# bghira/SimpleTuner

Measured on AMD Instinct MI355X. Metric: training images/sec (whole node), Flux.1-dev LoRA r32 1024^2 train step, higher is better.
Workload: dtype bf16

## Files before the change

### simpletuner_amd/csrc/gemm.hip

```cpp
#include <stdlib.h>
#include <type_traits>
#include "common.h"

#define BK 64
#define EPI_SPLITK 100

#ifdef ST355_TRACE
#define TR_T0 40
#define TR_MARKS 12
__device__ uint64_t st355_trace_buf[2][TR_MARKS];
#define TR_DECL uint64_t tr_[TR_MARKS] = {}
#define TR(t, k)                                                  \
  do {                                                            \
    if ((t) == TR_T0) tr_[k] = __builtin_amdgcn_s_memtime();       \
  } while (0)
#define TR_FLUSH(wv, lane)                                                              \
  do {                                                                                  \
    if (blockIdx.x == 64 && (lane) == 0 && ((wv) & 3) == 0)                              \
      for (int k_ = 0; k_ < TR_MARKS; k_++) st355_trace_buf[(wv) >> 2][k_] = tr_[k_];    \
  } while (0)
#else
#define TR_DECL
#define TR(t, k)
#define TR_FLUSH(wv, lane)
// ... 605 lines not shown
#define P3_THREADS 512
#define P3_XBYTES (P3_BM * BK * 2)
#define P3_WBYTES (P3_BN * BK * 2)
#define P3_STAGE (P3_XBYTES + P3_WBYTES)
#define P3_LDS (3 * P3_STAGE)

template <int EPI>
__global__ void __launch_bounds__(P3_THREADS, 2) k_gemm_p3(GemmGroup g) {
  extern __shared__ __attribute__((aligned(16))) char smem[];
  const int tid = threadIdx.x;
  const int lane = tid & 63;
  const int wv = __builtin_amdgcn_readfirstlane(tid >> 6);
  const int wm = wv >> 1, wn = wv & 1;

  int id = xcd_remap(blockIdx.x, gridDim.x);
  const int pi = id >= g.tiles0 ? 1 : 0;
  if (pi) id -= g.tiles0;
  const GemmP& p0 = g.p[pi];
  const int nbm = (p0.M + P3_BM - 1) / P3_BM, nbn = (p0.N + P3_BN - 1) / P3_BN;
  int pm, pn;
  tile_coords(id, nbm, nbn, pm, pn);
  const int m0 = pm * P3_BM, n0 = pn * P3_BN;
  const GemmP p = seg_view(p0, m0);
  const int nt1 = p.K / BK;
  const int nt = nt1 + p.K2 / BK;

  const bf16* A1 = p.A; const bf16* B1 = p.B; const bf16* A2 = p.A2; const bf16* B2 = p.B2;
  const int64_t la2 = p.lda2, lb2 = p.ldb2;
  const int M = p.M, N = p.N;
  const int st_row = lane >> 3, st_cp = lane & 7;
  int64_t xo[4], wo[2];
  int xrow[4], wrow[2], xc[4], wc[2];
#pragma unroll
  for (int j = 0; j < 4; j++) {
    const int row = (wv * 4 + j) * 8 + st_row;
    xc[j] = (st_cp ^ ((row >> 1) & 7)) * 8;
    xrow[j] = min(m0 + row, M - 1);
    xo[j] = (int64_t)xrow[j] * p.lda + xc[j];
  }
#pragma unroll
  for (int j = 0; j < 2; j++) {
    const int row = (wv * 2 + j) * 8 + st_row;
    wc[j] = (st_cp ^ ((row >> 1) & 7)) * 8;
    wrow[j] = min(n0 + row, N - 1);
    wo[j] = (int64_t)wrow[j] * p.ldb + wc[j];
  }
  auto stage = [&](int t, int buf) {
    char* xs = smem + buf * P3_STAGE;
    char* ws = xs + P3_XBYTES;
    if (t < nt1) {
      const int k0 = t * BK;
#pragma unroll
      for (int j = 0; j < 4; j++) glds16(A1 + xo[j] + k0, xs + (wv * 4 + j) * 1024);
#pragma unroll
      for (int j = 0; j < 2; j++) glds16(B1 + wo[j] + k0, ws + (wv * 2 + j) * 1024);
    } else {
      const int k0 = (t - nt1) * BK;
#pragma unroll
      for (int j = 0; j < 4; j++) glds16(A2 + (int64_t)xrow[j] * la2 + xc[j] + k0, xs + (wv * 4 + j) * 1024);
#pragma unroll
      for (int j = 0; j < 2; j++) glds16(B2 + (int64_t)wrow[j] * lb2 + wc[j] + k0, ws + (wv * 2 + j) * 1024);
    }
  };

  int w_off[2], w_sw[2], x_off[2], x_sw[2];
#pragma unroll
  for (int i = 0; i < 2; i++) {
    const int wr = wn * 64 + i * 32 + (lane & 31);
    w_off[i] = wr * 128; w_sw[i] = (wr >> 1) & 7;
    const int xr = wm * 64 + i * 32 + (lane & 31);
    x_off[i] = xr * 128; x_sw[i] = (xr >> 1) & 7;
  }
  const int khalf = lane >> 5;
  f32x16 acc[2][2];
#pragma unroll
  for (int i = 0; i < 2; i++)
#pragma unroll
    for (int j = 0; j < 2; j++)
#pragma unroll
      for (int r = 0; r < 16; r++) acc[i][j][r] = 0.f;

  stage(0, 0);
  if (nt > 1) {
    stage(1, 1);
    asm volatile("s_waitcnt vmcnt(6)" ::: "memory");
  } else {
    asm volatile("s_waitcnt vmcnt(0)" ::: "memory");
  }
  __builtin_amdgcn_s_barrier();
  int cur = 0;
  for (int t = 0; t < nt; t++) {
    if (t + 2 < nt) stage(t + 2, cur == 0 ? 2 : cur - 1);
    const char* xs = smem + cur * P3_STAGE;
    mma_tile(xs, xs + P3_XBYTES, x_off, x_sw, w_off, w_sw, khalf, acc);
    if (t + 1 < nt) {
      if (t + 2 < nt) asm volatile("s_waitcnt vmcnt(6)" ::: "memory");
      else asm volatile("s_waitcnt vmcnt(0)" ::: "memory");
      asm volatile("s_waitcnt lgkmcnt(0)" ::: "memory");
      __builtin_amdgcn_s_barrier();
    }
    cur = (cur == 2) ? 0 : cur + 1;
  }
  gemm_epilogue<EPI>(p, acc, m0 + wm * 64, n0 + wn * 64, lane);
}

#define PP_BARRIER()                                   \
  do {                                                 \
    asm volatile("" ::: "memory");                     \
    __builtin_amdgcn_s_barrier();                      \
    asm volatile("" ::: "memory");                     \
  } while (0)

#define PQ_BM 256
#define PQ_BN 256
#define PQ_BK 64
#define PQ_THREADS 512
#define PQ_REGION 16384
#define PQ_BUF (4 * PQ_REGION)
#define PQ_LDS (8 * 64 * 272)
#ifndef PQ_BUFLD
#define PQ_BUFLD 1
#endif
#ifndef PQ_VM
#define PQ_VM 8
#endif
#ifndef PQ_ABL
#define PQ_ABL 0
#endif
#ifndef PQ_PRIO
#ifndef PQ_F8_MX
#define PQ_F8_MX 1
#endif
typedef int i32x8 __attribute__((ext_vector_type(8)));
__device__ __forceinline__ i32x8 frag32(const long* p) {
  i32x8 v;
#pragma unroll
  for (int q = 0; q < 4; q++) { v[2 * q] = (int)(p[q] & 0xffffffffl); v[2 * q + 1] = (int)(p[q] >> 32); }
  return v;
}
#define PQ_PRIO 1
#endif
#ifndef PQ_GL
#define PQ_GL 1
#endif

__device__ __forceinline__ void wait_vm_rt(int n) {
  if (n >= 8) asm volatile("s_waitcnt vmcnt(8)" ::: "memory");
  else if (n == 6) asm volatile("s_waitcnt vmcnt(6)" ::: "memory");
  else if (n == 4) asm volatile("s_waitcnt vmcnt(4)" ::: "memory");
  else if (n == 2) asm volatile("s_waitcnt vmcnt(2)" ::: "memory");
  else asm volatile("s_waitcnt vmcnt(0)" ::: "memory");
}

template <int EPI, bool TN, bool F8 = false, bool CONV = false, int SK = 0>
__global__ void __launch_bounds__(PQ_THREADS, 2) k_gemm_pq(GemmGroup g) {
  static_assert(!SK || (!TN && !F8 && !CONV && EPI != EPI_SPLITK), "the stream-K tail is built for the plain NT bf16 problems");
  constexpr int ES = F8 ? 1 : 2;
  constexpr int KSN = F8 ? 8 : 4;
  static_assert(!(F8 && TN), "fp8 weight gradients are not built");
  extern __shared__ __attribute__((aligned(16))) char smem[];
  const int tid = threadIdx.x;
  const int lane = tid & 63;
  const int wv = __builtin_amdgcn_readfirstlane(tid >> 6);
  const int wm = wv >> 2, wn = wv & 3;

  int slice = (EPI == EPI_SPLITK) ? blockIdx.x / g.tiles0 : 0;
  int id = (EPI == EPI_SPLITK) ? xcd_remap(blockIdx.x % g.tiles0, g.tiles0) : xcd_remap(blockIdx.x, SK ? min((int)gridDim.x, g.sk_first) : (int)gridDim.x);
  int sk_n = 1, sk_tl = 0;
  if (SK && (int)blockIdx.x >= g.sk_first) {
    const int l = blockIdx.x - g.sk_first;
    sk_n = SK;
    const int lq = __builtin_amdgcn_readfirstlane((l >> 3) / sk_n);
    slice = (l >> 3) - lq * sk_n;
    sk_tl = 8 * lq + (l & 7);
    if (sk_tl >= g.tiles0 - g.sk_first) return;
    id = g.sk_first + sk_tl;
  }
  const int pi = id >= g.tiles0 ? 1 : 0;
  if (pi) id -= g.tiles0;
  const GemmP& p = g.p[pi];
  const int nbm = (p.M + PQ_BM - 1) / PQ_BM, nbn = (p.N + PQ_BN - 1) / PQ_BN;
  const int wtaps = (TN && p.conv_taps == 9) ? 9 : 1;
  int pm, pn;
  tile_coords(id, nbm, nbn * wtaps, pm, pn, TN ? ST355_TILE_GROUP : tile_group_for(p.K + p.K2));
  const int wtap = pn / nbn;
  pn -= wtap * nbn;
  const int m0 = pm * PQ_BM, n0 = pn * PQ_BN;
  const int64_t segi = (!TN && !F8 && !CONV && p.seg_rows) ? __builtin_amdgcn_readfirstlane(m0 / p.seg_rows) : 0;
  const int nt_all = p.K / (PQ_BK * 2 / ES);
  const int per = (EPI == EPI_SPLITK) ? (nt_all + p.ksplit - 1) / p.ksplit : SK ? __builtin_amdgcn_readfirstlane((nt_all + sk_n - 1) / sk_n) : nt_all;
  const int t_first = slice * per;
  const int nt1 = (EPI == EPI_SPLITK || SK) ? max(0, min(nt_all, t_first + per) - t_first) : nt_all;
  const int nt = nt1 + ((EPI == EPI_SPLITK || (SK && slice != sk_n - 1)) ? 0 : p.K2 / PQ_BK);

  const bf16* A1 = p.A + segi * p.seg_xa; const bf16* B1 = p.B; const bf16* A2 = p.A2 + segi * p.seg_xa2; const bf16* B2 = p.B2;
  const int64_t la2 = p.lda2, lb2 = p.ldb2;
  const int M = p.M, N = p.N;
  const char* xbase = TN ? (const char*)A1 + (int64_t)m0 * 2 : (const char*)A1 + (int64_t)m0 * p.lda * ES;
  const char* wbase = TN ? (const char*)B1 + (int64_t)n0 * 2 + (int64_t)((wtap / 3) * p.conv_wp + (wtap % 3)) * (wtaps > 1 ? p.ldb * 2 : 0)
                         : (const char*)B1 + (int64_t)n0 * p.ldb * ES;
  const uint32_t lda_b = (uint32_t)p.lda * ES, ldb_b = (uint32_t)p.ldb * ES;
  const int64_t xk_step = TN ? (int64_t)PQ_BK * lda_b : PQ_BK * 2;
  const int64_t wk_step = TN ? (int64_t)PQ_BK * ldb_b : PQ_BK * 2;
  constexpr bool conv = CONV;
  static_assert(!(CONV && (TN || F8)), "conv mode is the NT bf16 form");
  if (!conv) xbase += t_first * xk_step;
  wbase += t_first * wk_step;

  auto x_rel = [&](int lr, int r) { return min(m0 + (lr >> 6) * 128 + (lr & 63) + r * 64, M - 1) - m0; };
  auto w_rel = [&](int lr, int r) { return min(n0 + (lr >> 5) * 64 + (lr & 31) + r * 32, N - 1) - n0; };
  uint32_t xo[2][2], wo[2][2];
#pragma unroll
  for (int j = 0; j < 2; j++) {
    if (TN) {
      const int r4 = (wv * 2 + j) * 4 + (lane >> 4);
      const int cs = (lane & 15) ^ ((r4 & 3) << 2);
#pragma unroll
      for (int r = 0; r < 2; r++) {
        const int xc = min(m0 + (cs >> 3) * 128 + (cs & 7) * 8 + r * 64, M - 8) - m0;
        const int wc = min(n0 + (cs >> 2) * 64 + (cs & 3) * 8 + r * 32, N - 8) - n0;
        xo[r][j] = (uint32_t)r4 * lda_b + (uint32_t)(xc * 2);
        wo[r][j] = (uint32_t)r4 * ldb_b + (uint32_t)(wc * 2);
      }
    } else {
      const int lr = (wv * 2 + j) * 8 + (lane >> 3);
      const uint32_t scb = (uint32_t)(((lane & 7) ^ ((lr >> 1) & 7)) * 16);
#pragma unroll
      for (int r = 0; r < 2; r++) {
        xo[r][j] = (uint32_t)x_rel(lr, r) * lda_b + scb;
        wo[r][j] = (uint32_t)w_rel(lr, r) * ldb_b + scb;
      }
    }
  }
  auto stage_ext = [&](const bf16* base, int64_t ld, int row0, bool is_x, int r, int k0, char* dst) {
#pragma unroll
    for (int j = 0; j < 2; j++) {
      const int lr = (wv * 2 + j) * 8 + (lane >> 3);
      const int rel = is_x ? x_rel(lr, r) : w_rel(lr, r);
      glds16(base + (int64_t)(row0 + rel) * ld + ((lane & 7) ^ ((lr >> 1) & 7)) * 8 + k0, dst + j * 1024);
    }
  };
  const auto x_rsrc = __builtin_amdgcn_make_buffer_rsrc((void*)xbase, 0, 0x7FFFFFFF, 0x00020000);
  const auto w_rsrc = __builtin_amdgcn_make_buffer_rsrc((void*)wbase, 0, 0x7FFFFFFF, 0x00020000);
  auto stage_x = [&](int u, int r) {
    char* dst = smem + (u & 1) * PQ_BUF + r * PQ_REGION + wv * 2048;
    if (u < nt1) {
      const int x_ko = conv ? (int)(conv_koff(p, u + t_first, p.lda, PQ_BK) * 2)
                            : (int)(u * xk_step) + (TN ? (int)__umulhi((uint32_t)(u + t_first), p.tn_magic) * p.tn_skip_a : 0);
      if (PQ_BUFLD) {
#pragma unroll
        for (int j = 0; j < 2; j++)
          __builtin_amdgcn_raw_ptr_buffer_load_lds(x_rsrc, (__attribute__((address_space(3))) void*)(dst + j * 1024), 16, xo[r][j], x_ko, 0, 0);
        return;
      }
      const char* kb = xbase + x_ko;
#pragma unroll
      for (int j = 0; j < 2; j++) glds16((const bf16*)(kb + xo[r][j]), dst + j * 1024);
    } else {
      stage_ext(A2, la2, m0, true, r, (u - nt1) * PQ_BK, dst);
    }
  };
  auto stage_w = [&](int u, int r) {
    char* dst = smem + (u & 1) * PQ_BUF + (2 + r) * PQ_REGION + wv * 2048;
    if (u < nt1) {
      const int w_ko = (int)(u * wk_step) + (TN ? (int)__umulhi((uint32_t)(u + t_first), p.tn_magic) * p.tn_skip_b : 0);
      if (PQ_BUFLD) {
#pragma unroll
        for (int j = 0; j < 2; j++)
          __builtin_amdgcn_raw_ptr_buffer_load_lds(w_rsrc, (__attribute__((address_space(3))) void*)(dst + j * 1024), 16, wo[r][j], w_ko, 0, 0);
        return;
      }
      const char* kb = wbase + w_ko;
#pragma unroll
      for (int j = 0; j < 2; j++) glds16((const bf16*)(kb + wo[r][j]), dst + j * 1024);
    } else {
      stage_ext(B2, lb2, n0, false, r, (u - nt1) * PQ_BK, dst);
    }
  };
  auto refill = [&](int t, int ph, bool check) {
    if (PQ_ABL & 2) return;
    if (ph == 0) { if (!check || t + 1 < nt) stage_w(t + 1, 1); }
    else if (ph == 1) { if (!check || t + 1 < nt) stage_x(t + 1, 1); }
    else if (ph == 2) { if (!check || t + 2 < nt) stage_x(t + 2, 0); }
    else { if (!check || t + 2 < nt) stage_w(t + 2, 0); }
  };

  const int khalf = lane >> 5;
  const int l31 = lane & 31;
  int xk[4], wk[4];
#pragma unroll
  for (int ks = 0; ks < 4; ks++) {
    const int ch = ((2 * ks + khalf) ^ ((l31 >> 1) & 7)) << 4;
    xk[ks] = (wm * 64 + l31) * 128 + ch;
    wk[ks] = 2 * PQ_REGION + (wn * 32 + l31) * 128 + ch;
  }
  const int tg = lane >> 4, tti = (lane >> 2) & 3, tts = lane & 3;
  const int t_row = (8 * (tg >> 1) + tti) * 256 + (tts & 1) * 8;
  const int xt = t_row + (((wm * 8 + 2 * (tg & 1) + (tts >> 1)) ^ (tti << 2)) << 4);
  const int wt = 2 * PQ_REGION + t_row + (((wn * 4 + 2 * (tg & 1) + (tts >> 1)) ^ (tti << 2)) << 4);
  int xk8[8], wk8[8];
#pragma unroll
  for (int ks = 0; ks < 8; ks++) {
    const int chunk = PQ_F8_MX ? 4 * (ks >> 2) + 2 * khalf + ((ks & 3) >> 1) : ks;
    const int half8 = PQ_F8_MX ? (ks & 1) : khalf;
    const int ch = ((chunk ^ ((l31 >> 1) & 7)) << 4) + half8 * 8;
    xk8[ks] = (wm * 64 + l31) * 128 + ch;
    wk8[ks] = 2 * PQ_REGION + (wn * 32 + l31) * 128 + ch;
  }
  auto ld_x8 = [&](const char* base, int j, int ks) -> long { return *(const long*)(base + xk8[ks] + j * 4096); };
  auto ld_w8 = [&](const char* base, int ks) -> long { return *(const long*)(base + wk8[ks]); };
  auto ld_x = [&](const char* base, int j, int ks) -> bf16x8 {
    if (PQ_ABL & 1) { bf16x8 z; for (int q_ = 0; q_ < 8; q_++) z[q_] = (bf16)(float)(lane + j + ks); asm volatile("" : "+v"(z)); return z; }
    if (TN) { const char* q = base + (xt ^ (j << 6)) + ks * 4096; return lds_tr16x2(q, q + 1024); }
    return *(const bf16x8*)(base + xk[ks] + j * 4096);
  };
  auto ld_w = [&](const char* base, int ks) -> bf16x8 {
    if (PQ_ABL & 1) { bf16x8 z; for (int q_ = 0; q_ < 8; q_++) z[q_] = (bf16)(float)(lane + ks); asm volatile("" : "+v"(z)); return z; }
    if (TN) { const char* q = base + wt + ks * 4096; return lds_tr16x2(q, q + 1024); }
    return *(const bf16x8*)(base + wk[ks]);
  };
  f32x16 acc[2][4];
#pragma unroll
  for (int i = 0; i < 2; i++)
#pragma unroll
    for (int j = 0; j < 4; j++)
#pragma unroll
      for (int r = 0; r < 16; r++) acc[i][j][r] = 0.f;

  stage_x(0, 0); stage_w(0, 0); stage_w(0, 1); stage_x(0, 1);
  if (nt > 1) { stage_x(1, 0); stage_w(1, 0); }
  if (PQ_ABL & 2) wait_vm_rt(0); else
  wait_vm_rt(nt > 1 ? 8 : 4);
  PP_BARRIER();
  if (wm == 1) PP_BARRIER();

  bf16x8 xf[2][4], w0f[4], w1f[4];
  long xf8[2][8], w0f8[8], w1f8[8];
  const bool mma_live = !CONV || !p.skip_dead || (n0 + wn * 64 < N);
  TR_DECL;
#define PQ_MMA(WF, I, J0, T, PH)                                                                              \
  do {                                                                                                        \
    if (PQ_PRIO) __builtin_amdgcn_s_setprio(1);                                                               \
    if (F8 && PQ_F8_MX) {                                                                                     \
      _Pragma("unroll") for (int s2 = 0; s2 < 2; s2++)                                                        \
        _Pragma("unroll") for (int j = 0; j < 2; j++)                                                         \
          acc[I][J0 + j] = __builtin_amdgcn_mfma_scale_f32_32x32x64_f8f6f4(frag32(&WF##8[4 * s2]), frag32(&xf8[j][4 * s2]), acc[I][J0 + j], \
                                                                            0 , 1 , 0, 0x7f7f7f7f, 0, 0x7f7f7f7f); \
    } else if (F8) {                                                                                          \
      _Pragma("unroll") for (int ks = 0; ks < 8; ks++)                                                        \
        _Pragma("unroll") for (int j = 0; j < 2; j++)                                                         \
          acc[I][J0 + j] = __builtin_amdgcn_mfma_f32_32x32x16_fp8_bf8(WF##8[ks], xf8[j][ks], acc[I][J0 + j], 0, 0, 0); \
    } else if (!CONV || mma_live)                                                                             \
    _Pragma("unroll") for (int ks = 0; ks < 4; ks++) {                                                        \
      _Pragma("unroll") for (int j = 0; j < 2; j++)                                                           \
        acc[I][J0 + j] = __builtin_amdgcn_mfma_f32_32x32x16_bf16(WF[ks], xf[j][ks], acc[I][J0 + j], 0, 0, 0); \
      if (PQ_GL == 3 && ks == 1) { __builtin_amdgcn_sched_barrier(0); refill(T, PH, TAIL); __builtin_amdgcn_sched_barrier(0); } \
    }                                                                                                         \
    if (PQ_PRIO) __builtin_amdgcn_s_setprio(0);                                                               \
  } while (0)

  auto body = [&](int t, auto tail_c) {
    constexpr bool TAIL = decltype(tail_c)::value;
    const char* bf = smem + (t & 1) * PQ_BUF;
    const int rem = nt - 1 - t;
    TR(t, 0);
    if (PQ_GL == 0) refill(t, 0, TAIL);
#pragma unroll
    for (int j = 0; j < 2; j++)
#pragma unroll
      for (int ks = 0; ks < KSN; ks++) { if (F8) xf8[j][ks] = ld_x8(bf, j, ks); else xf[j][ks & 3] = ld_x(bf, j, ks & 3); }
#pragma unroll
    for (int ks = 0; ks < KSN; ks++) { if (F8) w0f8[ks] = ld_w8(bf, ks); else w0f[ks & 3] = ld_w(bf, ks & 3); }
    if (PQ_GL == 1) refill(t, 0, TAIL);
    TR(t, 1);
    if (!TAIL) wait_vm_rt(PQ_VM); else wait_vm_rt(rem >= 2 ? 8 : (rem == 1 ? 8 : 2));
    PP_BARRIER();
    TR(t, 2);
    PQ_MMA(w0f, 0, 0, t, 1);
    if (PQ_GL == 2) refill(t, 1, TAIL);
    TR(t, 3);
    PP_BARRIER();
    if (PQ_GL == 0) refill(t, 1, TAIL);
#pragma unroll
    for (int ks = 0; ks < KSN; ks++) { if (F8) w1f8[ks] = ld_w8(bf + PQ_REGION, ks); else w1f[ks & 3] = ld_w(bf + PQ_REGION, ks & 3); }
    if (PQ_GL == 1) refill(t, 1, TAIL);
    TR(t, 4);
    if (!TAIL) wait_vm_rt(PQ_VM); else wait_vm_rt(rem >= 2 ? 8 : (rem == 1 ? 8 : 0));
    PP_BARRIER();
    TR(t, 5);
    PQ_MMA(w1f, 1, 0, t, 2);
    if (PQ_GL == 2) refill(t, 2, TAIL);
    TR(t, 6);
    PP_BARRIER();
    if (PQ_GL == 0) refill(t, 2, TAIL);
#pragma unroll
    for (int j = 0; j < 2; j++)
#pragma unroll
      for (int ks = 0; ks < KSN; ks++) { if (F8) xf8[j][ks] = ld_x8(bf + PQ_REGION, j, ks); else xf[j][ks & 3] = ld_x(bf + PQ_REGION, j, ks & 3); }
    if (PQ_GL == 1) refill(t, 2, TAIL);
    TR(t, 7);
    if (!TAIL) wait_vm_rt(PQ_VM); else wait_vm_rt(rem >= 2 ? 8 : (rem == 1 ? 6 : 0));
    PP_BARRIER();
    TR(t, 8);
    PQ_MMA(w1f, 1, 2, t, 3);
    if (PQ_GL == 2) refill(t, 3, TAIL);
    TR(t, 9);
    PP_BARRIER();
    if (PQ_GL == 0) refill(t, 3, TAIL);
    if (PQ_GL == 1) refill(t, 3, TAIL);
    if (!TAIL) wait_vm_rt(PQ_VM); else wait_vm_rt(rem >= 2 ? 8 : (rem == 1 ? 4 : 0));
    PP_BARRIER();
    TR(t, 10);
    PQ_MMA(w0f, 0, 2, t + 1, 0);
    if (PQ_GL == 2) refill(t + 1, 0, TAIL);
    TR(t, 11);
    PP_BARRIER();
  };
  if (PQ_GL == 2 || PQ_GL == 3) refill(0, 0, true);
  int t = 0;
  for (; t < nt - 2; t++) body(t, std::false_type{});
  for (; t < nt; t++) body(t, std::true_type{});
#undef PQ_MMA
  TR_FLUSH(wv, lane);
  if (wm == 0) PP_BARRIER();
  if (SK && sk_n > 1) {
    float* slab = g.sk_ws + ((int64_t)sk_tl * (sk_n - 1)) * (PQ_BM * PQ_BN) + tid * 4;
    int* flag = g.sk_flags + sk_tl;
    if (slice < sk_n - 1) {
      slab += (int64_t)slice * (PQ_BM * PQ_BN);
#pragma unroll
      for (int i = 0; i < 2; i++)
#pragma unroll
        for (int j = 0; j < 4; j++)
#pragma unroll
          for (int a = 0; a < 4; a++) {
            f32x4 v;
#pragma unroll
            for (int b = 0; b < 4; b++) v[b] = acc[i][j][4 * a + b];
            *(f32x4*)(slab + ((i * 4 + j) * 4 + a) * (PQ_THREADS * 4)) = v;
          }
      asm volatile("s_waitcnt vmcnt(0)" ::: "memory");
      __syncthreads();
      if (tid == 0) __hip_atomic_fetch_add(flag, 1, __ATOMIC_RELAXED, __HIP_MEMORY_SCOPE_AGENT);
      return;
    }
    if (tid == 0)
      while (__hip_atomic_load(flag, __ATOMIC_RELAXED, __HIP_MEMORY_SCOPE_AGENT) < sk_n - 1) __builtin_amdgcn_s_sleep(4);
    __syncthreads();
    asm volatile("" ::: "memory");
#pragma unroll
    for (int i = 0; i < 2; i++)
#pragma unroll
      for (int j = 0; j < 4; j++) {
        f32x4 v[SK > 1 ? SK - 1 : 1][4];
#pragma unroll
        for (int k = 0; k < SK - 1; k++)
#pragma unroll
          for (int a = 0; a < 4; a++) v[k][a] = *(const f32x4*)(slab + (int64_t)k * (PQ_BM * PQ_BN) + ((i * 4 + j) * 4 + a) * (PQ_THREADS * 4));
#pragma unroll
        for (int k = 0; k < SK - 1; k++)
#pragma unroll
          for (int a = 0; a < 4; a++)
#pragma unroll
            for (int b = 0; b < 4; b++) acc[i][j][4 * a + b] += v[k][a][b];
        asm volatile("" ::: "memory");
      }
    if (tid == 0) __hip_atomic_store(flag, 0, __ATOMIC_RELAXED, __HIP_MEMORY_SCOPE_AGENT);
  }
  if (EPI == EPI_SPLITK) {
    GemmP ps = p;
    ps.partial = p.partial + (int64_t)slice * p.M * p.part_ld + (int64_t)wtap * p.N;
    ps.bias = nullptr;
    ps.conv_taps = 0;
    gemm_epilogue_lds<EPI, false, false>(ps, acc, m0 + wm * 128, n0 + wn * 64, lane, smem + wv * EPL_WAVE);
  } else if (wtaps > 1) {
    GemmP ps = p;
    ps.C = p.C + (int64_t)wtap * p.N;
    if (ps.aux_in) ps.aux_in = p.aux_in + (int64_t)wtap * p.N;
    ps.conv_taps = 0;
    gemm_epilogue_lds<EPI, false, false>(ps, acc, m0 + wm * 128, n0 + wn * 64, lane, smem + wv * EPL_WAVE);
  } else if (EPI == ST355_EPI_HEADS) {
    gemm_epilogue_heads(p, p.C + segi * p.seg_xc, acc, m0 + wm * 128, n0 + wn * 64, lane, smem + wv * EPL_WAVE);
  } else if (EPI == ST355_EPI_GEGLU) {
    gemm_epilogue_geglu(p, acc, m0 + wm * 128, n0 + wn * 64, lane, smem + wv * EPL_WAVE);
  } else if (EPI == ST355_EPI_GEGLU_GRAD) {
    gemm_epilogue_geglu_grad(p, acc, m0 + wm * 128, n0 + wn * 64, lane, smem + wv * EPL_WAVE);
  } else if (EPI == ST355_EPI_QK_NORM_ROPE) {
    if (n0 >= 2 * p.rH * 128) {
      gemm_epilogue_vdual(p, p.C + segi * p.seg_xc, acc, m0, n0, wm, wn, wv, lane, smem);
    } else {
      gemm_epilogue_qkrope(p, acc, m0, n0, wm, wn, wv, lane, smem);
    }
  } else if (!TN && !F8 && !CONV) {
    GemmP ps = p;
    ps.C = p.C + segi * p.seg_xc;
    ps.aux_in = p.aux_in + segi * p.seg_xin;
    ps.aux_out = p.aux_out + segi * p.seg_xout;
    if (epl_aligned(ps)) gemm_epilogue_lds<EPI, false, false>(ps, acc, m0 + wm * 128, n0 + wn * 64, lane, smem + wv * EPL_WAVE);
    else gemm_epilogue<EPI, 2, 4>(ps, acc, m0 + wm * 128, n0 + wn * 64, lane);
  } else if (epl_aligned(p)) gemm_epilogue_lds<EPI, CONV, F8>(p, acc, m0 + wm * 128, n0 + wn * 64, lane, smem + wv * EPL_WAVE);
  else gemm_epilogue<EPI, 2, 4>(p, acc, m0 + wm * 128, n0 + wn * 64, lane);
}

#define PZ_LDS (2 * PQ_BUF + 32768)
#define PZ_STAGE 8192

template <int EPI>
__device__ __forceinline__ void gemm_epilogue_lds8(const GemmP& p, f32x16 (&acc)[2][4], int mw0, int nw0, int lane, char* stage) {
  const int khalf = lane >> 5, l31 = lane & 31;
  const int rrow = lane >> 3, rc = lane & 7;
  const int n = nw0 + rc * 8;
  float bias8[8];
#pragma unroll
  for (int b = 0; b < 8; b++) bias8[b] = 0.f;
  if (p.bias) {
    const bf16x8 bv = *(const bf16x8*)(p.bias + n);
#pragma unroll
    for (int b = 0; b < 8; b++) bias8[b] = bf2f(bv[b]);
  }
  const int m_first = mw0 + rrow;
  constexpr bool GG = EPI == ST355_EPI_GEGLU_GRAD;
  const int nc = GG ? 2 * nw0 + 64 * (rc >> 2) + (rc & 3) * 8 : n;
  bf16* c_row = p.C + (int64_t)m_first * p.ldc + nc;
  const bf16* in_row = p.aux_in ? p.aux_in + (int64_t)m_first * p.ld_aux_in + nc : nullptr;
  bf16* out_row = p.aux_out ? p.aux_out + (int64_t)m_first * p.ld_aux_out + n : nullptr;
  const int64_t c_step = 8 * p.ldc, in_step = 8 * p.ld_aux_in, out_step = 8 * p.ld_aux_out;
  typedef __attribute__((address_space(3))) char lds_char;
  typedef __attribute__((address_space(3))) f32x4 lds_f32x4;
  const uint32_t stage_u = (uint32_t)(uintptr_t)(lds_char*)stage;
  const uint32_t wbase0 = stage_u + (uint32_t)(l31 * 256 + ((khalf ^ (l31 & 15)) << 4));
  const uint32_t rb = stage_u + (uint32_t)(rrow * 256);
  const uint32_t r_lo_e = rb + (uint32_t)((((2 * rc) ^ rrow)) << 4), r_hi_e = rb + (uint32_t)((((2 * rc + 1) ^ rrow)) << 4);
  const uint32_t r_lo_o = rb + (uint32_t)((((2 * rc) ^ (rrow | 8))) << 4), r_hi_o = rb + (uint32_t)((((2 * rc + 1) ^ (rrow | 8))) << 4);
  constexpr bool AUXIN = (EPI == ST355_EPI_GATE_RESIDUAL || EPI == ST355_EPI_ADD || EPI == ST355_EPI_MUL_GELU_GRAD || GG);
  bf16x8 auxv[2][4], gatev[2][4];
  const bf16* in_pre = in_row;
  int m_pre = m_first;
  auto preload = [&](bf16x8 (&av)[4], bf16x8 (&gv)[4]) {
#pragma unroll
    for (int it = 0; it < 4; it++) {
      if (AUXIN) av[it] = *(const bf16x8*)in_pre;
      if (EPI == ST355_EPI_GATE_RESIDUAL) gv[it] = *(const bf16x8*)(p.gate + (int64_t)(m_pre / p.rows_per_batch) * p.gate_stride + n);
      if (GG) gv[it] = *(const bf16x8*)(in_pre + 32);
      in_pre += in_step; m_pre += 8;
    }
  };
  if (AUXIN) preload(auxv[0], gatev[0]);
#pragma unroll
  for (int j = 0; j < 4; j++) {
    uint32_t wb = wbase0;
    asm volatile("" : "+v"(wb));
#pragma unroll
    for (int i = 0; i < 2; i++)
#pragma unroll
      for (int a = 0; a < 4; a++) {
        f32x4 v;
#pragma unroll
        for (int b = 0; b < 4; b++) v[b] = acc[i][j][4 * a + b];
        *(lds_f32x4*)(wb ^ (uint32_t)((i * 8 + 2 * a) << 4)) = v;
      }
    if (AUXIN && j < 3) preload(auxv[(j + 1) & 1], gatev[(j + 1) & 1]);
#pragma unroll
    for (int it = 0; it < 4; it++) {
      const f32x4 lo = *(const lds_f32x4*)(((it & 1) ? r_lo_o : r_lo_e) + (uint32_t)(it * 2048));
      const f32x4 hi = *(const lds_f32x4*)(((it & 1) ? r_hi_o : r_hi_e) + (uint32_t)(it * 2048));
      bf16* const c_ptr = c_row;
      bf16* const out_ptr = out_row;
      c_row += c_step; out_row += out_step;
      float v[8];
#pragma unroll
      for (int b = 0; b < 4; b++) { v[b] = lo[b] + bias8[b]; v[4 + b] = hi[b] + bias8[4 + b]; }
      if (EPI == ST355_EPI_GELU) {
        if (p.aux_out) {
          bf16x8 pre;
#pragma unroll
          for (int b = 0; b < 8; b++) pre[b] = f2bf(v[b]);
          *(bf16x8*)out_ptr = pre;
#pragma unroll
          for (int b = 0; b < 8; b++) v[b] = bf2f(pre[b]);
        }
#pragma unroll
        for (int b = 0; b < 8; b++) v[b] = gelu_tanh(v[b]);
      } else if (EPI == ST355_EPI_GATE_RESIDUAL) {
        if (p.aux_out) {
          bf16x8 yv;
#pragma unroll
          for (int b = 0; b < 8; b++) yv[b] = f2bf(v[b]);
          *(bf16x8*)out_ptr = yv;
        }
        const bf16x8 gv = gatev[j & 1][it];
        const bf16x8 rv = auxv[j & 1][it];
#pragma unroll
        for (int b = 0; b < 8; b++) v[b] = bf2f(rv[b]) + bf2f(gv[b]) * v[b];
      } else if (EPI == ST355_EPI_ADD) {
        const bf16x8 rv = auxv[j & 1][it];
#pragma unroll
        for (int b = 0; b < 8; b++) v[b] += bf2f(rv[b]);
      } else if (EPI == ST355_EPI_MUL_GELU_GRAD) {
        const bf16x8 hv = auxv[j & 1][it];
#pragma unroll
        for (int b = 0; b < 8; b++) v[b] *= gelu_tanh_grad(bf2f(hv[b]));
      }
      if (GG) {
        const bf16x8 vv = auxv[j & 1][it], gv = gatev[j & 1][it];
        bf16x8 dv, dg;
#pragma unroll
        for (int b = 0; b < 8; b++) {
          const float d = bf2f(f2bf(v[b]));
          const float g = bf2f(gv[b]);
          dv[b] = f2bf(d * gelu_erf(g));
          dg[b] = f2bf(d * bf2f(vv[b]) * gelu_erf_grad(g));
        }
        *(bf16x8*)c_ptr = dv;
        *(bf16x8*)(c_ptr + 32) = dg;
        continue;
      }
      bf16x8 o;
#pragma unroll
      for (int b = 0; b < 8; b++) o[b] = f2bf(v[b]);
      *(bf16x8*)c_ptr = o;
    }
  }
}

template <int EPI>
__global__ void __launch_bounds__(PQ_THREADS, 2) k_gemm_pz(GemmP p, int ntiles) {
  extern __shared__ __attribute__((aligned(16))) char smem[];
  const int tid = threadIdx.x;
  const int lane = tid & 63;
  const int wv = __builtin_amdgcn_readfirstlane(tid >> 6);
  const int wm = wv >> 2, wn = wv & 3;
  const int nbm = p.M / PQ_BM, nbn = p.N / PQ_BN;
  const int nt1 = p.K / PQ_BK;
  const int nt = nt1 + p.K2 / PQ_BK;
  const int G = gridDim.x;
  const uint32_t lda_b = (uint32_t)p.lda * 2, ldb_b = (uint32_t)p.ldb * 2;
  const int64_t la2 = p.lda2, lb2 = p.ldb2;

  struct Tile { int m0, n0; const char* xb; const char* wb; const bf16* a2; const bf16* b2; int64_t segi; };
  auto tile_at = [&](int id) {
    Tile t;
    int pm, pn;
    tile_coords(id, nbm, nbn, pm, pn);
    t.m0 = __builtin_amdgcn_readfirstlane(pm * PQ_BM);
    t.n0 = __builtin_amdgcn_readfirstlane(pn * PQ_BN);
    t.segi = p.seg_rows ? (int64_t)__builtin_amdgcn_readfirstlane(t.m0 / p.seg_rows) : 0;
    t.xb = (const char*)(p.A + t.segi * p.seg_xa) + (int64_t)t.m0 * lda_b;
    t.wb = (const char*)p.B + (int64_t)t.n0 * ldb_b;
    t.a2 = p.A2 + t.segi * p.seg_xa2 + (int64_t)t.m0 * la2;
    t.b2 = p.B2 + (int64_t)t.n0 * lb2;
    return t;
  };

  int tile_id = xcd_remap(blockIdx.x, G);
  Tile cur = tile_at(tile_id);
  int par = 0;
  bool first = true;

  while (true) {
    int ln = lane;
    asm volatile("" : "+v"(ln));
    uint32_t xo[2][2], wo[2][2];
#pragma unroll
    for (int j = 0; j < 2; j++) {
      const int lr = (wv * 2 + j) * 8 + (ln >> 3);
      const uint32_t scb = (uint32_t)(((ln & 7) ^ ((lr >> 1) & 7)) * 16);
#pragma unroll
      for (int r = 0; r < 2; r++) {
        xo[r][j] = (uint32_t)((lr >> 6) * 128 + (lr & 63) + r * 64) * lda_b + scb;
        wo[r][j] = (uint32_t)((lr >> 5) * 64 + (lr & 31) + r * 32) * ldb_b + scb;
      }
    }
    const int khalf = ln >> 5;
    const int l31 = ln & 31;
    int xk[4], wk[4];
#pragma unroll
    for (int ks = 0; ks < 4; ks++) {
      const int ch = ((2 * ks + khalf) ^ ((l31 >> 1) & 7)) << 4;
      xk[ks] = (wm * 64 + l31) * 128 + ch;
      wk[ks] = 2 * PQ_REGION + (wn * 32 + l31) * 128 + ch;
    }
    auto ld_x = [&](const char* base, int j, int ks) -> bf16x8 { return *(const bf16x8*)(base + xk[ks] + j * 4096); };
    auto ld_w = [&](const char* base, int ks) -> bf16x8 { return *(const bf16x8*)(base + wk[ks]); };
    const bool has_next = tile_id + G < ntiles;
    const Tile nxt = has_next ? tile_at(tile_id + G) : cur;
    const auto x_rsrc = __builtin_amdgcn_make_buffer_rsrc((void*)cur.xb, 0, 0x7FFFFFFF, 0x00020000);
    const auto w_rsrc = __builtin_amdgcn_make_buffer_rsrc((void*)cur.wb, 0, 0x7FFFFFFF, 0x00020000);
    const auto xn_rsrc = __builtin_amdgcn_make_buffer_rsrc((void*)nxt.xb, 0, 0x7FFFFFFF, 0x00020000);
    const auto wn_rsrc = __builtin_amdgcn_make_buffer_rsrc((void*)nxt.wb, 0, 0x7FFFFFFF, 0x00020000);

    auto stage_x = [&](int u, int r, int mode) {
      char* dst = smem + (((u & 1) ^ par) * PQ_BUF) + r * PQ_REGION + wv * 2048;
      const bool nx = mode == 1 && u >= nt;
      const int uu = nx ? u - nt : u;
      if (uu < nt1) {
#pragma unroll
        for (int j = 0; j < 2; j++)
          __builtin_amdgcn_raw_ptr_buffer_load_lds(nx ? xn_rsrc : x_rsrc, (__attribute__((address_space(3))) void*)(dst + j * 1024), 16, xo[r][j], uu * (PQ_BK * 2), 0, 0);
      } else {
        const bf16* base = nx ? nxt.a2 : cur.a2;
#pragma unroll
        for (int j = 0; j < 2; j++) {
          const int lr = (wv * 2 + j) * 8 + (ln >> 3);
          glds16(base + (int64_t)((lr >> 6) * 128 + (lr & 63) + r * 64) * la2 + ((ln & 7) ^ ((lr >> 1) & 7)) * 8 + (uu - nt1) * PQ_BK, dst + j * 1024);
        }
      }
    };
    auto stage_w = [&](int u, int r, int mode) {
      char* dst = smem + (((u & 1) ^ par) * PQ_BUF) + (2 + r) * PQ_REGION + wv * 2048;
      const bool nx = mode == 1 && u >= nt;
      const int uu = nx ? u - nt : u;
      if (uu < nt1) {
#pragma unroll
        for (int j = 0; j < 2; j++)
          __builtin_amdgcn_raw_ptr_buffer_load_lds(nx ? wn_rsrc : w_rsrc, (__attribute__((address_space(3))) void*)(dst + j * 1024), 16, wo[r][j], uu * (PQ_BK * 2), 0, 0);
      } else {
        const bf16* base = nx ? nxt.b2 : cur.b2;
#pragma unroll
        for (int j = 0; j < 2; j++) {
          const int lr = (wv * 2 + j) * 8 + (ln >> 3);
          glds16(base + (int64_t)((lr >> 5) * 64 + (lr & 31) + r * 32) * lb2 + ((ln & 7) ^ ((lr >> 1) & 7)) * 8 + (uu - nt1) * PQ_BK, dst + j * 1024);
        }
      }
    };
    auto refill = [&](int t, int ph, int mode) {
      const int u = (ph < 2) ? t + 1 : t + 2;
      if (mode == 2 && u >= nt) return;
      if (ph == 0) stage_w(u, 1, mode);
      else if (ph == 1) stage_x(u, 1, mode);
      else if (ph == 2) stage_x(u, 0, mode);
      else stage_w(u, 0, mode);
    };

    f32x16 acc[2][4];
#pragma unroll
    for (int i = 0; i < 2; i++)
#pragma unroll
      for (int j = 0; j < 4; j++)
#pragma unroll
        for (int r = 0; r < 16; r++) acc[i][j][r] = 0.f;

    if (first) {
      stage_x(0, 0, 0); stage_w(0, 0, 0); stage_w(0, 1, 0); stage_x(0, 1, 0);
      stage_x(1, 0, 0); stage_w(1, 0, 0);
      wait_vm_rt(8);
      PP_BARRIER();
    }
    if (wm == 1) PP_BARRIER();

    bf16x8 xf[2][4], w0f[4], w1f[4];
#define PZ_MMA(WF, I, J0)                                                                                     \
  do {                                                                                                        \
    __builtin_amdgcn_s_setprio(1);                                                                            \
    _Pragma("unroll") for (int ks = 0; ks < 4; ks++)                                                          \
      _Pragma("unroll") for (int j = 0; j < 2; j++)                                                           \
        acc[I][J0 + j] = __builtin_amdgcn_mfma_f32_32x32x16_bf16(WF[ks], xf[j][ks], acc[I][J0 + j], 0, 0, 0); \
    __builtin_amdgcn_s_setprio(0);                                                                            \
  } while (0)

    auto body = [&](int t, auto mode_c, auto firstk_c) {
      constexpr int MODE = decltype(mode_c)::value;
      constexpr bool FIRSTK = decltype(firstk_c)::value;
      const char* bf = smem + (((t & 1) ^ par) * PQ_BUF);
      const int rem = nt - 1 - t;
#pragma unroll
      for (int j = 0; j < 2; j++)
#pragma unroll
        for (int ks = 0; ks < 4; ks++) xf[j][ks] = ld_x(bf, j, ks);
#pragma unroll
      for (int ks = 0; ks < 4; ks++) w0f[ks] = ld_w(bf, ks);
      refill(t, 0, MODE);
      if (MODE != 2) { if (!FIRSTK) wait_vm_rt(8); } else wait_vm_rt(rem >= 1 ? 8 : 2);
      PP_BARRIER();
      PZ_MMA(w0f, 0, 0);
      PP_BARRIER();
#pragma unroll
      for (int ks = 0; ks < 4; ks++) w1f[ks] = ld_w(bf + PQ_REGION, ks);
      refill(t, 1, MODE);
      if (MODE != 2) { if (!FIRSTK) wait_vm_rt(8); } else wait_vm_rt(rem >= 1 ? 8 : 0);
      PP_BARRIER();
      PZ_MMA(w1f, 1, 0);
      PP_BARRIER();
#pragma unroll
      for (int j = 0; j < 2; j++)
#pragma unroll
        for (int ks = 0; ks < 4; ks++) xf[j][ks] = ld_x(bf + PQ_REGION, j, ks);
      refill(t, 2, MODE);
      if (MODE != 2) wait_vm_rt(8); else wait_vm_rt(rem >= 1 ? 6 : 0);
      PP_BARRIER();
      PZ_MMA(w1f, 1, 2);
      PP_BARRIER();
      refill(t, 3, MODE);
      if (MODE != 2) wait_vm_rt(8); else wait_vm_rt(rem >= 1 ? 4 : 0);
      PP_BARRIER();
      PZ_MMA(w0f, 0, 2);
      PP_BARRIER();
    };
    int t = 0;
    if (!first) { body(0, std::integral_constant<int, 0>{}, std::true_type{}); t = 1; }
    for (; t < nt - 2; t++) body(t, std::integral_constant<int, 0>{}, std::false_type{});
    for (; t < nt; t++) body(t, std::integral_constant<int, 1>{}, std::false_type{});
#undef PZ_MMA
    if (wm == 0) PP_BARRIER();
    wait_vm_rt(4);
    {
      GemmP ps = p;
      ps.C = p.C + cur.segi * p.seg_xc;
      ps.aux_in = p.aux_in ? p.aux_in + cur.segi * p.seg_xin : nullptr;
      ps.aux_out = p.aux_out ? p.aux_out + cur.segi * p.seg_xout : nullptr;
      char* const lastbuf = smem + ((((nt - 1) & 1) ^ par) * PQ_BUF);
      char* const stg = wv < 2 ? lastbuf + PQ_REGION + wv * PZ_STAGE : (wv < 4 ? lastbuf + 3 * PQ_REGION + (wv - 2) * PZ_STAGE : smem + 2 * PQ_BUF + (wv - 4) * PZ_STAGE);
      int le = lane;
      asm volatile("" : "+v"(le));
      gemm_epilogue_lds8<EPI>(ps, acc, cur.m0 + wm * 128, cur.n0 + wn * 64, le, stg);
    }
    if (!has_next) { wait_vm_rt(0); break; }
    PP_BARRIER();
    par ^= (nt & 1);
    tile_id += G;
    cur = nxt;
    first = false;
  }
}

#define S2_BM 128
#define S2_BN 128
#define S2_THREADS 256
#define S2_TILE (128 * BK * 2)
#define S2_STAGE (2 * S2_TILE)
#define S2_LDS (2 * S2_STAGE)

template <int EPI>
__global__ void __launch_bounds__(S2_THREADS, 2) k_gemm_s2(GemmP p_in) {
  extern __shared__ __attribute__((aligned(16))) char smem[];
  const int tid = threadIdx.x;
  const int lane = tid & 63;
  const int wv = __builtin_amdgcn_readfirstlane(tid >> 6);
  const int wm = wv >> 1, wn = wv & 1;
  const int nbm = (p_in.M + S2_BM - 1) / S2_BM, nbn = (p_in.N + S2_BN - 1) / S2_BN;
  int pm, pn;
  const int tiles = nbm * nbn;
  const int slice = (EPI == EPI_SPLITK) ? blockIdx.x / tiles : 0;
  tile_coords(xcd_remap((EPI == EPI_SPLITK) ? blockIdx.x % tiles : blockIdx.x, tiles), nbm, nbn, pm, pn);
  const int m0 = pm * S2_BM, n0 = pn * S2_BN;
  const GemmP p = seg_view(p_in, m0);
  const int nt1 = p.K / BK;
  const int per = (EPI == EPI_SPLITK) ? (nt1 + p.ksplit - 1) / p.ksplit : 0;
  const int t_first = (EPI == EPI_SPLITK) ? slice * per : 0;
  const int nt = (EPI == EPI_SPLITK) ? min(nt1, t_first + per) : nt1 + p.K2 / BK;
  const int st_row = lane >> 3, st_cp = lane & 7;
  auto stage = [&](int t, int buf) {
    const bf16* Ap; const bf16* Bp; int64_t la, lb; int k0;
    if (t < nt1) { Ap = p.A; la = p.lda; Bp = p.B; lb = p.ldb; k0 = t * BK; }
    else { Ap = p.A2; la = p.lda2; Bp = p.B2; lb = p.ldb2; k0 = (t - nt1) * BK; }
    const int64_t ka = (p.conv_taps && t < nt1) ? conv_koff(p, t, la, BK) : (int64_t)k0;
    char* xs = smem + buf * S2_STAGE;
    char* ws = xs + S2_TILE;
#pragma unroll
    for (int j = 0; j < 4; j++) {
      const int r0 = (wv * 4 + j) * 8;
      const int row = r0 + st_row;
      const int c = st_cp ^ ((row >> 1) & 7);
      glds16(Ap + (int64_t)min(m0 + row, p.M - 1) * la + ka + c * 8, xs + r0 * 128);
      glds16(Bp + (int64_t)min(n0 + row, p.N - 1) * lb + k0 + c * 8, ws + r0 * 128);
    }
  };
  int w_off[2], w_sw[2], x_off[2], x_sw[2];
#pragma unroll
  for (int i = 0; i < 2; i++) {
    const int wr = wn * 64 + i * 32 + (lane & 31);
    w_off[i] = wr * 128; w_sw[i] = (wr >> 1) & 7;
    const int xr = wm * 64 + i * 32 + (lane & 31);
    x_off[i] = xr * 128; x_sw[i] = (xr >> 1) & 7;
  }
  const int khalf = lane >> 5;
  f32x16 acc[2][2];
#pragma unroll
  for (int i = 0; i < 2; i++)
#pragma unroll
    for (int j = 0; j < 2; j++)
#pragma unroll
      for (int r = 0; r < 16; r++) acc[i][j][r] = 0.f;
  if (t_first < nt) stage(t_first, 0);
  __syncthreads();
  for (int t = t_first; t < nt; t++) {
    const int buf = (t - t_first) & 1;
    if (t + 1 < nt) stage(t + 1, buf ^ 1);
    const char* xs = smem + buf * S2_STAGE;
    mma_tile(xs, xs + S2_TILE, x_off, x_sw, w_off, w_sw, khalf, acc);
    __syncthreads();
  }
  if (EPI == EPI_SPLITK) {
    float* slab = p.partial + (int64_t)slice * p.M * p.N;
#pragma unroll
    for (int j = 0; j < 2; j++) {
      const int m = m0 + wm * 64 + j * 32 + (lane & 31);
      if (m >= p.M) continue;
#pragma unroll
      for (int i = 0; i < 2; i++)
#pragma unroll
        for (int a = 0; a < 4; a++) {
          const int n = n0 + wn * 64 + i * 32 + 8 * a + 4 * khalf;
          if (n >= p.N) continue;
          f32x4 v;
#pragma unroll
          for (int b = 0; b < 4; b++) v[b] = acc[i][j][4 * a + b];
          *(f32x4*)(slab + (int64_t)m * p.N + n) = v;
        }
    }
  } else {
    gemm_epilogue<(EPI == EPI_SPLITK) ? ST355_EPI_NONE : EPI>(p, acc, m0 + wm * 64, n0 + wn * 64, lane);
  }
}

__global__ void __launch_bounds__(256) k_splitk_reduce(const float* __restrict__ slabs, int ksplit, const bf16* __restrict__ bias,
                                                      bf16* __restrict__ C, int64_t ldc, int M, int N, int accumulate) {
  const int64_t i4 = (int64_t)blockIdx.x * blockDim.x + threadIdx.x;
  const int n4 = N / 4;
  if (i4 >= (int64_t)M * n4) return;
  const int m = (int)(i4 / n4), n = (int)(i4 % n4) * 4;
  f32x4 s = *(const f32x4*)(slabs + (int64_t)m * N + n);
  for (int k = 1; k < ksplit; k++) {
    const f32x4 v = *(const f32x4*)(slabs + ((int64_t)k * M + m) * N + n);
    s += v;
  }
  bf16x4 o;
#pragma unroll
  for (int b = 0; b < 4; b++) o[b] = f2bf(s[b] + (bias ? bf2f(bias[n + b]) : 0.f));
  if (accumulate) {
    const bf16x4 c0 = *(const bf16x4*)(C + (int64_t)m * ldc + n);
#pragma unroll
    for (int b = 0; b < 4; b++) o[b] = f2bf(s[b] + bf2f(c0[b]));
  }
  *(bf16x4*)(C + (int64_t)m * ldc + n) = o;
}

static int validate(const st355_gemm_args* a) {
  ST_REQUIRE(a && a->A && a->B && a->C, "gemm: null pointer");
  ST_REQUIRE(a->M > 0 && a->N > 0 && a->K > 0, "gemm: empty shape M=%d N=%d K=%d", a->M, a->N, a->K);
  ST_REQUIRE(a->K % BK == 0 && a->K2 % BK == 0, "gemm: K (%d) and K2 (%d) must be multiples of 64", a->K, a->K2);
  ST_REQUIRE(a->N % 4 == 0 && a->ldc % 4 == 0, "gemm: N (%d) and ldc must be multiples of 4", a->N);
  ST_REQUIRE(a->lda % 8 == 0 && a->ldb % 8 == 0, "gemm: lda/ldb must be multiples of 8 (16-byte rows)");
  ST_REQUIRE(((uintptr_t)a->A % 16 == 0) && ((uintptr_t)a->B % 16 == 0) && ((uintptr_t)a->C % 8 == 0), "gemm: misaligned pointer");
  if (a->K2 > 0) {
    ST_REQUIRE(a->A2 && a->B2 && a->lda2 % 8 == 0 && a->ldb2 % 8 == 0, "gemm: low-rank extension operands missing/misaligned");
    ST_REQUIRE(((uintptr_t)a->A2 % 16 == 0) && ((uintptr_t)a->B2 % 16 == 0), "gemm: misaligned A2/B2");
  }
  if (a->epilogue == ST355_EPI_GATE_RESIDUAL)
    ST_REQUIRE(a->gate && a->aux_in && a->rows_per_batch > 0 && a->gate_stride % 4 == 0 && a->ld_aux_in % 4 == 0,
               "gemm: gate/residual epilogue operands missing");
  if (a->epilogue == ST355_EPI_MUL_GELU_GRAD || a->epilogue == ST355_EPI_ADD)
    ST_REQUIRE(a->aux_in && a->ld_aux_in % 4 == 0, "gemm: gelu-grad/add epilogue needs aux_in");
  if ((a->epilogue == ST355_EPI_GELU || a->epilogue == ST355_EPI_GATE_RESIDUAL) && a->aux_out)
    ST_REQUIRE(a->ld_aux_out % 4 == 0, "gemm: ld_aux_out must be a multiple of 4");
  ST_REQUIRE(a->epilogue >= 0 && a->epilogue <= ST355_EPI_HEADS, "gemm: unknown epilogue %d", a->epilogue);
  if (a->epilogue == ST355_EPI_HEADS) {
    const st355_heads* h = a->heads;
// ... 928 lines not shown
```

Measured before the change: 6.258.

## Switch bf16 NT GEMM inner loop from 32x32x16 to 16x16x32 MFMA

Replaces the 32x32x16 bf16 MFMA tiles in the plain NT bf16 and persistent GEMM paths with 16x16x32 MFMAs. It remaps the LDS fragment offsets to suit the new shape and adds a permlane16 swap before the epilogue so accumulators return to the layout the epilogue expects. The aim is higher matrix-core throughput or better LDS read patterns on MI355X. In exchange it issues more MFMA instructions per K step and adds a permute cost at the epilogue.

```diff
diff --git a/simpletuner_amd/csrc/gemm.hip b/simpletuner_amd/csrc/gemm.hip
--- a/simpletuner_amd/csrc/gemm.hip
+++ b/simpletuner_amd/csrc/gemm.hip
@@ -781,6 +781,48 @@
   else asm volatile("s_waitcnt vmcnt(0)" ::: "memory");
 }
 
+__device__ __forceinline__ void pq_frag16(int lane, int xbase, int wbase, int (&xk)[4], int (&wk)[4]) {
+  const int l15 = lane & 15, kq = lane >> 4;
+  const int w15 = (l15 & 3) | ((l15 & 4) << 1) | ((l15 & 8) >> 1);
+#pragma unroll
+  for (int q = 0; q < 4; q++) {
+    const int tile = q >> 1, ks = q & 1;
+    xk[q] = xbase + (16 * tile + l15) * 128 + (((4 * ks + kq) ^ ((l15 >> 1) & 7)) << 4);
+    wk[q] = wbase + (16 * tile + w15) * 128 + (((4 * ks + kq) ^ ((w15 >> 1) & 7)) << 4);
+  }
+}
+__device__ __forceinline__ void pq_mma16(f32x16& acc0, f32x16& acc1, const bf16x8 (&wf)[4], const bf16x8 (&xf)[2][4], int ks) {
+#pragma unroll
+  for (int fi = 0; fi < 2; fi++)
+#pragma unroll
+    for (int j = 0; j < 2; j++)
+#pragma unroll
+      for (int tj = 0; tj < 2; tj++) {
+        f32x16& acc = j ? acc1 : acc0;
+        const int r0 = 8 * fi + 4 * tj;
+        f32x4 c;
+#pragma unroll
+        for (int b = 0; b < 4; b++) c[b] = acc[r0 + b];
+        c = __builtin_amdgcn_mfma_f32_16x16x32_bf16(wf[2 * fi + ks], xf[j][2 * tj + ks], c, 0, 0, 0);
+#pragma unroll
+        for (int b = 0; b < 4; b++) acc[r0 + b] = c[b];
+      }
+}
+__device__ __forceinline__ void pq_acc_swap16(f32x16 (&acc)[2][4]) {
+#pragma unroll
+  for (int i = 0; i < 2; i++)
+#pragma unroll
+    for (int j = 0; j < 4; j++)
+#pragma unroll
+      for (int fi = 0; fi < 2; fi++)
+#pragma unroll
+        for (int b = 0; b < 4; b++) {
+          const auto r = __builtin_amdgcn_permlane16_swap(__float_as_uint(acc[i][j][8 * fi + b]), __float_as_uint(acc[i][j][8 * fi + 4 + b]), false, false);
+          acc[i][j][8 * fi + b] = __uint_as_float(r[0]);
+          acc[i][j][8 * fi + 4 + b] = __uint_as_float(r[1]);
+        }
+}
+
 template <int EPI, bool TN, bool F8 = false, bool CONV = false, int SK = 0>
 __global__ void __launch_bounds__(PQ_THREADS, 2) k_gemm_pq(GemmGroup g) {
   static_assert(!SK || (!TN && !F8 && !CONV && EPI != EPI_SPLITK), "the stream-K tail is built for the plain NT bf16 problems");
@@ -914,14 +956,18 @@
     else { if (!check || t + 2 < nt) stage_w(t + 2, 0); }
   };
 
+  constexpr bool M16 = !TN && !F8 && !CONV;
   const int khalf = lane >> 5;
   const int l31 = lane & 31;
-  int xk[4], wk[4];
-#pragma unroll
-  for (int ks = 0; ks < 4; ks++) {
-    const int ch = ((2 * ks + khalf) ^ ((l31 >> 1) & 7)) << 4;
-    xk[ks] = (wm * 64 + l31) * 128 + ch;
-    wk[ks] = 2 * PQ_REGION + (wn * 32 + l31) * 128 + ch;
+  int xk[4] = {}, wk[4] = {};
+  if (M16) pq_frag16(lane, wm * 64 * 128, 2 * PQ_REGION + wn * 32 * 128, xk, wk);
+  else if (CONV) {
+#pragma unroll
+    for (int ks = 0; ks < 4; ks++) {
+      const int ch = ((2 * ks + khalf) ^ ((l31 >> 1) & 7)) << 4;
+      xk[ks] = (wm * 64 + l31) * 128 + ch;
+      wk[ks] = 2 * PQ_REGION + (wn * 32 + l31) * 128 + ch;
+    }
   }
   const int tg = lane >> 4, tti = (lane >> 2) & 3, tts = lane & 3;
   const int t_row = (8 * (tg >> 1) + tti) * 256 + (tts & 1) * 8;
@@ -979,7 +1025,12 @@
       _Pragma("unroll") for (int ks = 0; ks < 8; ks++)                                                        \
         _Pragma("unroll") for (int j = 0; j < 2; j++)                                                         \
           acc[I][J0 + j] = __builtin_amdgcn_mfma_f32_32x32x16_fp8_bf8(WF##8[ks], xf8[j][ks], acc[I][J0 + j], 0, 0, 0); \
-    } else if (!CONV || mma_live)                                                                             \
+    } else if (M16) {                                                                                         \
+      _Pragma("unroll") for (int ks = 0; ks < 2; ks++) {                                                      \
+        pq_mma16(acc[I][J0], acc[I][J0 + 1], WF, xf, ks);                                                     \
+        if (PQ_GL == 3 && ks == 0) { __builtin_amdgcn_sched_barrier(0); refill(T, PH, TAIL); __builtin_amdgcn_sched_barrier(0); } \
+      }                                                                                                       \
+    } else if (!CONV || mma_live)                                                \
     _Pragma("unroll") for (int ks = 0; ks < 4; ks++) {                                                        \
       _Pragma("unroll") for (int j = 0; j < 2; j++)                                                           \
         acc[I][J0 + j] = __builtin_amdgcn_mfma_f32_32x32x16_bf16(WF[ks], xf[j][ks], acc[I][J0 + j], 0, 0, 0); \
@@ -1096,6 +1147,7 @@
       }
     if (tid == 0) __hip_atomic_store(flag, 0, __ATOMIC_RELAXED, __HIP_MEMORY_SCOPE_AGENT);
   }
+  if (M16) pq_acc_swap16(acc);
   if (EPI == EPI_SPLITK) {
     GemmP ps = p;
     ps.partial = p.partial + (int64_t)slice * p.M * p.part_ld + (int64_t)wtap * p.N;
@@ -1300,15 +1352,8 @@
         wo[r][j] = (uint32_t)((lr >> 5) * 64 + (lr & 31) + r * 32) * ldb_b + scb;
       }
     }
-    const int khalf = ln >> 5;
-    const int l31 = ln & 31;
     int xk[4], wk[4];
-#pragma unroll
-    for (int ks = 0; ks < 4; ks++) {
-      const int ch = ((2 * ks + khalf) ^ ((l31 >> 1) & 7)) << 4;
-      xk[ks] = (wm * 64 + l31) * 128 + ch;
-      wk[ks] = 2 * PQ_REGION + (wn * 32 + l31) * 128 + ch;
-    }
+    pq_frag16(ln, wm * 64 * 128, 2 * PQ_REGION + wn * 32 * 128, xk, wk);
     auto ld_x = [&](const char* base, int j, int ks) -> bf16x8 { return *(const bf16x8*)(base + xk[ks] + j * 4096); };
     auto ld_w = [&](const char* base, int ks) -> bf16x8 { return *(const bf16x8*)(base + wk[ks]); };
     const bool has_next = tile_id + G < ntiles;
@@ -1381,9 +1426,7 @@
 #define PZ_MMA(WF, I, J0)                                                                                     \
   do {                                                                                                        \
     __builtin_amdgcn_s_setprio(1);                                                                            \
-    _Pragma("unroll") for (int ks = 0; ks < 4; ks++)                                                          \
-      _Pragma("unroll") for (int j = 0; j < 2; j++)                                                           \
-        acc[I][J0 + j] = __builtin_amdgcn_mfma_f32_32x32x16_bf16(WF[ks], xf[j][ks], acc[I][J0 + j], 0, 0, 0); \
+    _Pragma("unroll") for (int ks = 0; ks < 2; ks++) pq_mma16(acc[I][J0], acc[I][J0 + 1], WF, xf, ks);        \
     __builtin_amdgcn_s_setprio(0);                                                                            \
   } while (0)
 
@@ -1432,6 +1475,7 @@
 #undef PZ_MMA
     if (wm == 0) PP_BARRIER();
     wait_vm_rt(4);
+    pq_acc_swap16(acc);
     {
       GemmP ps = p;
       ps.C = p.C + cur.segi * p.seg_xc;
```

Measured after the change: 6.382 (median of 6 runs). +2.0%, better.
